# szcompressor/sz

Measured on AMD Instinct MI355X. Metric: compression GB/s (input), 512^3 float32 ABS 1e-4, higher is better.
Workload: dtype f32

## Files before the change

### sz_amd/csrc/szh_segenc.h

```cpp
#pragma once

namespace szh_se {
constexpr int NR = 4;
constexpr int INNER = 7;
constexpr int PF = 8;

struct col_t { int b0, b1, s0, s1, o0, o1, rows; };
struct seg_t {
    int bkbeg, bkend, kbeg, kend;
    int nE, E, L;
    int ka, nvec, pitch, kshift;
    int nblk, nruns;
    int lg_nvec;
};
SZH_HD int seg_pitch(int width) { int p = (width + 1) & ~1; if (((p >> 1) & 1) == 0) p += 2; return p; }
SZH_HD col_t make_col(const szh_geom3 &G, int col)
{
    col_t c;
    c.b0 = col / G.g1.num; c.b1 = col - c.b0 * G.g1.num;
    c.s0 = szh_blk_size(G.g0, c.b0); c.s1 = szh_blk_size(G.g1, c.b1); c.o0 = szh_blk_start(G.g0, c.b0); c.o1 = szh_blk_start(G.g1, c.b1);
    c.rows = c.s0 * c.s1;
    return c;
}
SZH_HD seg_t make_seg(const szh_geom3 &G, int rows, int segi, int segb, int VW)
{
    seg_t s;
    s.bkbeg = segi * segb; s.bkend = s.bkbeg + segb < G.g2.num ? s.bkbeg + segb : G.g2.num;
    s.kbeg = szh_blk_start(G.g2, s.bkbeg); s.kend = s.bkend < G.g2.num ? szh_blk_start(G.g2, s.bkend) : G.g2.count;
    s.E = G.g2.early; s.L = G.g2.late;
    int nE = G.g2.split - s.bkbeg; if (nE < 0) nE = 0; if (nE > s.bkend - s.bkbeg) nE = s.bkend - s.bkbeg;
    s.nE = nE;
    s.ka = s.kbeg / VW * VW;
    const int kb = (s.kend + VW - 1) / VW * VW;
    s.nvec = (kb - s.ka) / VW;
    s.pitch = seg_pitch(kb - s.ka); s.kshift = s.kbeg - s.ka;
    s.nblk = s.bkend - s.bkbeg; s.nruns = s.nblk * rows;
    s.lg_nvec = 0; while ((1 << s.lg_nvec) < s.nvec) ++s.lg_nvec;
    return s;
}
inline size_t seg_tile_bytes(const szh_geom3 &G, int segb, int VW)
{
    const size_t rows = (size_t)G.g0.early * G.g1.early;
    const int width = segb * G.g2.early + 2 * VW;
    return (rows * (size_t)seg_pitch(width) * 2 + 15) & ~(size_t)15;
}
inline size_t seg_pieces_per_thread(const szh_geom3 &G, int segb, int VW)
{
    const size_t rows = (size_t)G.g0.early * G.g1.early;
    const size_t nvec = ((size_t)segb * G.g2.early + 2 * VW) / VW + 1;
    size_t p2 = 1; while (p2 < nvec) p2 <<= 1;
    return (rows * p2 + 255) / 256;
}
inline size_t seg_window_words(const szh_geom3 &G, unsigned maxlen, int nrmax = NR) { return (size_t)256 * nrmax * (size_t)G.g2.early * maxlen / 32 + 8; }
}

#ifdef SZH_HIPSIM
static inline bool any_lane(bool p) { return __ballot(p ? 1 : 0) != 0ull; }
#else
__device__ __forceinline__ bool any_lane(bool p) { return __builtin_amdgcn_ballot_w64(p) != 0ull; }
#endif
__device__ __forceinline__ unsigned magic_of(unsigned d) { return d > 1u ? 0xffffffffu / d + 1u : 0u; }
__device__ __forceinline__ unsigned div_by(unsigned x, unsigned d, unsigned m) { return d > 1u ? (unsigned)(((u64)x * m) >> 32) : x; }

#define SZH_COL_HBINS 256
__global__ __launch_bounds__(256) void k_col_hist(szh_geom3 G, const uint16_t *__restrict__ codes, unsigned nbins, int rshift, int vw, unsigned *__restrict__ col_hist)
{
    SZH_DYN_SMEM(smem);
    unsigned *sh = reinterpret_cast<unsigned *>(smem);
    const unsigned R = 1u << rshift;
    for (unsigned i = threadIdx.x; i < (nbins << rshift); i += 256) sh[i] = 0;
    __syncthreads();
    const szh_se::col_t c = szh_se::make_col(G, (int)blockIdx.x);
    const int nvec = G.g2.count / vw;
    const int lane = (int)threadIdx.x & 63, wid = (int)threadIdx.x >> 6;
    const unsigned rep = threadIdx.x & (R - 1);
    const unsigned m_s1 = magic_of((unsigned)c.s1);
    for (int x = lane; x < nvec; x += 64) {
        for (int r0 = wid; r0 < c.rows; r0 += 16) {
            uint4 w[4];
#pragma unroll
            for (int q = 0; q < 4; ++q) {
                const int r = r0 + 4 * q;
                w[q] = uint4{0u, 0u, 0u, 0u};
                if (r < c.rows) {
                    const int i = (int)div_by((unsigned)r, (unsigned)c.s1, m_s1), j = r - i * c.s1;
                    const uint16_t *src = codes + (int64_t)(c.o0 + i) * G.d0 + (int64_t)(c.o1 + j) * G.d1 + x * vw;
                    if (vw == 8) w[q] = *reinterpret_cast<const uint4 *>(src);
                    else if (vw == 4) { const uint2 t = *reinterpret_cast<const uint2 *>(src); w[q].x = t.x; w[q].y = t.y; }
                    else w[q].x = src[0];
                }
            }
#pragma unroll
            for (int q = 0; q < 4; ++q) {
                if (r0 + 4 * q < c.rows) {
                    const unsigned wv[4] = {w[q].x, w[q].y, w[q].z, w[q].w};
#pragma unroll
                    for (int e = 0; e < 8; ++e) if (e < vw) { const unsigned cd = (e & 1) ? wv[e >> 1] >> 16 : wv[e >> 1] & 0xffffu; atomicAdd(&sh[(cd << rshift) + rep], 1u); }
                }
            }
        }
    }
    __syncthreads();
    for (unsigned b = threadIdx.x; b < nbins; b += 256) {
        unsigned t = 0;
        for (unsigned q = 0; q < R; ++q) t += sh[(b << rshift) + q];
        col_hist[(size_t)blockIdx.x * nbins + b] = t;
    }
}
__global__ __launch_bounds__(256) void k_hist_reduce(const unsigned *__restrict__ col_hist, unsigned nbins, int64_t ncols, unsigned *__restrict__ hist)
{
    __shared__ unsigned acc[SZH_COL_HBINS];
    for (unsigned b = threadIdx.x; b < nbins; b += 256) acc[b] = 0;
    __syncthreads();
    const unsigned tpb = 256u / nbins > 0u ? 256u / nbins : 1u;
    if (threadIdx.x < tpb * nbins) {
        const unsigned bin = threadIdx.x % nbins, lane_col = threadIdx.x / nbins;
        unsigned t = 0;
        for (int64_t col = (int64_t)blockIdx.x * tpb + lane_col; col < ncols; col += (int64_t)gridDim.x * tpb) t += col_hist[(size_t)col * nbins + bin];
        if (t) atomicAdd(&acc[bin], t);
    }
    __syncthreads();
    for (unsigned b = threadIdx.x; b < nbins; b += 256) if (acc[b]) atomicAdd(&hist[b], acc[b]);
}
__global__ __launch_bounds__(256) void k_col_bits_h(const unsigned *__restrict__ col_hist, const uint8_t *__restrict__ len, unsigned nbins, int64_t ncols, u64 *__restrict__ col_bits, u64 *__restrict__ col_zeros)
{
    __shared__ uint8_t llen[SZH_COL_HBINS];
    for (unsigned i = threadIdx.x; i < nbins; i += 256) llen[i] = len[i];
    __syncthreads();
    const int64_t e = (int64_t)blockIdx.x * 256 + threadIdx.x;
    if (e >= ncols) return;
    const unsigned *h = col_hist + (size_t)e * nbins;
    u64 bits = 0;
    for (unsigned b = 0; b < nbins; ++b) bits += (u64)h[b] * llen[b];
    col_bits[e] = bits; col_zeros[e] = h[0];
}

// ... 21 lines not shown
                    const int i = (int)div_by((unsigned)r, (unsigned)c.s1, m_s1), j = r - i * c.s1;
                    const uint16_t *src = codes + (int64_t)(c.o0 + i) * G.d0 + (int64_t)(c.o1 + j) * G.d1 + x * vw;
                    if (vw == 8) w[q] = *reinterpret_cast<const uint4 *>(src);
                    else if (vw == 4) { const uint2 t = *reinterpret_cast<const uint2 *>(src); w[q].x = t.x; w[q].y = t.y; }
                    else w[q].x = src[0];
                }
            }
#pragma unroll
            for (int q = 0; q < 4; ++q) {
                if (r0 + 4 * q < c.rows) {
                    const unsigned wv[4] = {w[q].x, w[q].y, w[q].z, w[q].w};
#pragma unroll
                    for (int e = 0; e < 8; ++e) if (e < vw) {
                        const unsigned cd = (e & 1) ? wv[e >> 1] >> 16 : wv[e >> 1] & 0xffffu;
                        bits += tab_lds ? llen[cd] : len[cd]; zeros += cd == 0u ? 1u : 0u;
                    }
                }
            }
        }
    }
    bits = wave_sum_u64(bits); const u64 z = wave_sum_u64((u64)zeros);
    if (lane == 0) { red[wid] = bits; red[4 + wid] = z; }
    __syncthreads();
    if (threadIdx.x == 0) { col_bits[blockIdx.x] = red[0] + red[1] + red[2] + red[3]; col_zeros[blockIdx.x] = red[4] + red[5] + red[6] + red[7]; }
}

__global__ __launch_bounds__(256) void k_col_bounds(const u64 *__restrict__ col_bitoff, int64_t nent, const u64 *__restrict__ total_bits, u64 bit0, unsigned *out32)
{
    const int64_t e = (int64_t)blockIdx.x * 256 + threadIdx.x;
    if (e > nent) return;
    const u64 at = bit0 + (e < nent ? col_bitoff[e] : *total_bits);
    out32[at >> 5] = 0u;
    if (e == nent) out32[(at >> 5) + 1] = 0u;
}
#define SZH_COL_SCAN_PER 8
__global__ __launch_bounds__(1024) void k_col_scan(const u64 *__restrict__ col_bits, const u64 *__restrict__ col_zeros, int nent, u64 *__restrict__ col_bitoff, u64 *__restrict__ col_zoff,
                                                   u64 *total_bits, u64 *total_zeros, u64 bit0, unsigned *out32, const u64 *__restrict__ plan = nullptr)
{
    __shared__ u64 shb[16], shz[16];
    if (plan) { if (plan[SZH_PLAN_STATUS] != 0) return; bit0 = plan[SZH_PLAN_BIT0]; }
    const int tid = (int)threadIdx.x, lane = tid & 63, wid = tid >> 6;
    const int lo = tid * SZH_COL_SCAN_PER;
    u64 vb[SZH_COL_SCAN_PER], vz[SZH_COL_SCAN_PER];
#pragma unroll
    for (int q = 0; q < SZH_COL_SCAN_PER; ++q) { const bool in = lo + q < nent; vb[q] = in ? col_bits[lo + q] : 0ull; vz[q] = in ? col_zeros[lo + q] : 0ull; }
    u64 b = 0, z = 0;
#pragma unroll
    for (int q = 0; q < SZH_COL_SCAN_PER; ++q) { b += vb[q]; z += vz[q]; }
    u64 ib = b, iz = z;
    for (int o = 1; o < 64; o <<= 1) { const u64 tb = __shfl_up(ib, o, 64), tz = __shfl_up(iz, o, 64); if (lane >= o) { ib += tb; iz += tz; } }
    if (lane == 63) { shb[wid] = ib; shz[wid] = iz; }
    __syncthreads();
    u64 baseb = 0, basez = 0, totb = 0, totz = 0;
    for (int w = 0; w < 16; ++w) { if (w < wid) { baseb += shb[w]; basez += shz[w]; } totb += shb[w]; totz += shz[w]; }
    u64 rb = baseb + ib - b, rz = basez + iz - z;
#pragma unroll
    for (int q = 0; q < SZH_COL_SCAN_PER; ++q) {
        if (lo + q < nent) { col_bitoff[lo + q] = rb; col_zoff[lo + q] = rz; out32[(bit0 + rb) >> 5] = 0u; }
        rb += vb[q]; rz += vz[q];
    }
    if (tid == 0) { *total_bits = totb; *total_zeros = totz; out32[(bit0 + totb) >> 5] = 0u; out32[((bit0 + totb) >> 5) + 1] = 0u; }
}

__global__ __launch_bounds__(1024) void k_col_zscan(const unsigned *__restrict__ col_zeros, int nent, u64 *__restrict__ col_zoff, u64 *total_zeros)
{
    __shared__ u64 shz[16];
    const int tid = (int)threadIdx.x, lane = tid & 63, wid = tid >> 6;
    const int lo = tid * SZH_COL_SCAN_PER;
    u64 vz[SZH_COL_SCAN_PER], z = 0;
#pragma unroll
    for (int q = 0; q < SZH_COL_SCAN_PER; ++q) { vz[q] = lo + q < nent ? (u64)col_zeros[lo + q] : 0ull; z += vz[q]; }
    u64 iz = z;
    for (int o = 1; o < 64; o <<= 1) { const u64 tz = __shfl_up(iz, o, 64); if (lane >= o) iz += tz; }
    if (lane == 63) shz[wid] = iz;
    __syncthreads();
    u64 basez = 0, totz = 0;
    for (int w = 0; w < 16; ++w) { if (w < wid) basez += shz[w]; totz += shz[w]; }
    u64 rz = basez + iz - z;
#pragma unroll
    for (int q = 0; q < SZH_COL_SCAN_PER; ++q) { if (lo + q < nent) col_zoff[lo + q] = rz; rz += vz[q]; }
    if (tid == 0) *total_zeros = totz;
}

template <class T, bool WIDE>
__global__ __launch_bounds__(256) void k_col_encode(szh_geom3 G, const uint16_t *__restrict__ codes, const u64 *__restrict__ table, unsigned nsym, const szh_se::seg_t *__restrict__ segs, int nseg, int vw, int nrmax,
                                                    size_t tile_bytes, unsigned win_words, const u64 *__restrict__ col_bitoff, const u64 *__restrict__ col_zoff, u64 bit0,
                                                    unsigned *out32, const T *__restrict__ data, T *__restrict__ unpred, const u64 *__restrict__ plan = nullptr)
{
    using namespace szh_se;
    if (plan) { if (plan[SZH_PLAN_STATUS] != 0) return; bit0 = plan[SZH_PLAN_BIT0]; }
    SZH_DYN_SMEM(smem);
    __shared__ u64 sh[2][4];
    __shared__ unsigned rowbase[128];
    u64 *ltab = reinterpret_cast<u64 *>(smem);
    uint16_t *tile = reinterpret_cast<uint16_t *>(smem + ((size_t)nsym + 1) * 8);
    uint16_t *nullrun = reinterpret_cast<uint16_t *>(smem + ((size_t)nsym + 1) * 8 + tile_bytes);
    unsigned *win = reinterpret_cast<unsigned *>(smem + ((size_t)nsym + 1) * 8 + tile_bytes + 16);
    const int tid = (int)threadIdx.x, lane = tid & 63, wid = tid >> 6;
    const col_t c = make_col(G, (int)blockIdx.x);
    for (unsigned i = tid; i < nsym; i += 256) ltab[i] = table[i];
    if (tid == 0) ltab[nsym] = 0;
    if (tid < 8) nullrun[tid] = (uint16_t)nsym;
    for (unsigned w = tid; w < win_words; w += 256) win[w] = 0u;
    const unsigned m_rows = magic_of((unsigned)c.rows);
    if (tid < c.rows) { const int i = tid / c.s1, j = tid - i * c.s1; rowbase[tid] = (unsigned)((int64_t)(c.o0 + i) * G.d0 + (int64_t)(c.o1 + j) * G.d1); }
    __syncthreads();
    uint4 pf[PF];
    auto fetch = [&](const seg_t &s) {
        const int lg = s.lg_nvec, mask = (1 << lg) - 1;
#pragma unroll
        for (int p = 0; p < PF; ++p) {
            const int x = p * 256 + tid, r = x >> lg, cv = x & mask;
            pf[p] = uint4{0u, 0u, 0u, 0u};
            if (r < c.rows && cv < s.nvec) {
                const uint16_t *src = codes + (size_t)rowbase[r] + (unsigned)(s.ka + cv * vw);
                if (vw == 8) pf[p] = *reinterpret_cast<const uint4 *>(src);
                else if (vw == 4) { const uint2 t = *reinterpret_cast<const uint2 *>(src); pf[p].x = t.x; pf[p].y = t.y; }
                else pf[p].x = src[0];
            }
        }
    };
    auto place = [&](const seg_t &s) {
        const int lg = s.lg_nvec, mask = (1 << lg) - 1;
        auto put_piece = [&](int r, int cv, const uint4 &w) {
            uint16_t *dst = tile + r * s.pitch + cv * vw;
            if (vw == 8) { unsigned *d = reinterpret_cast<unsigned *>(dst); d[0] = w.x; d[1] = w.y; d[2] = w.z; d[3] = w.w; }
            else if (vw == 4) { unsigned *d = reinterpret_cast<unsigned *>(dst); d[0] = w.x; d[1] = w.y; }
            else dst[0] = (uint16_t)w.x;
        };
#pragma unroll
        for (int p = 0; p < PF; ++p) { const int x = p * 256 + tid, r = x >> lg, cv = x & mask; if (r < c.rows && cv < s.nvec) put_piece(r, cv, pf[p]); }
        for (int x = PF * 256 + tid; (x >> lg) < c.rows; x += 256) {
            const int r = x >> lg, cv = x & mask;
            if (cv >= s.nvec) continue;
            const uint16_t *src = codes + (size_t)rowbase[r] + (unsigned)(s.ka + cv * vw);
            uint4 w = {0u, 0u, 0u, 0u};
            if (vw == 8) w = *reinterpret_cast<const uint4 *>(src);
            else if (vw == 4) { const uint2 t = *reinterpret_cast<const uint2 *>(src); w.x = t.x; w.y = t.y; }
            else w.x = src[0];
            put_piece(r, cv, w);
        }
    };
    seg_t s = segs[0]; s.nruns = s.nblk * c.rows;
    fetch(s);
    const u64 col_bit = bit0 + col_bitoff[blockIdx.x];
    const u64 col_word = col_bit >> 5;
    const bool col_lead = (col_bit & 31u) != 0u;
    u64 bits_done = 0, zeros_done = col_zoff[blockIdx.x];
    const int null_at = (int)(nullrun - tile);
    int par = 0;
    for (int segi = 0; segi < nseg; ++segi) {
        place(s);
        __syncthreads();
        seg_t sn = s;
        if (segi + 1 < nseg) { sn = segs[segi + 1]; sn.nruns = sn.nblk * c.rows; fetch(sn); }
        const int nrounds = (s.nruns + 256 * nrmax - 1) / (256 * nrmax);
        const int nr = (s.nruns + 256 * nrounds - 1) / (256 * nrounds);
        const int edge_k = s.nE * s.E;
        auto run_words = [&](int at, unsigned (&wv)[4]) {
            const unsigned *w = reinterpret_cast<const unsigned *>(tile + (at & ~1));
            const unsigned w0 = w[0], w1 = w[1], w2 = w[2], w3 = w[3];
            const unsigned sft = (unsigned)(at & 1) << 4;
            wv[0] = (unsigned)((((u64)w1 << 32) | w0) >> sft); wv[1] = (unsigned)((((u64)w2 << 32) | w1) >> sft);
            wv[2] = (unsigned)((((u64)w3 << 32) | w2) >> sft); wv[3] = w3 >> sft;
        };
        for (int rd = 0; rd < nrounds; ++rd, par ^= 1) {
            const int q0 = (rd * 256 + tid) * nr;
            const int bl0 = (int)div_by((unsigned)q0, (unsigned)c.rows, m_rows), row0 = q0 - bl0 * c.rows;
            unsigned sum1 = 0;
            int jn = 0;
            unsigned need7 = 0;
            if (WIDE) {
                int bl = bl0, row = row0;
                for (int j = 0; j < nr; ++j) {
                    const bool on = q0 + j < s.nruns;
                    if (!any_lane(on)) break;
                    jn = j + 1;
                    const int s2 = bl < s.nE ? s.E : s.L, koff = bl < s.nE ? bl * s.E : edge_k + (bl - s.nE) * s.L;
                    unsigned wv[4];
                    run_words(on ? row * s.pitch + s.kshift + koff : null_at, wv);
                    const bool n7 = any_lane(on && s2 == INNER);
                    if (n7) need7 |= 1u << j;
#pragma unroll
                    for (int kk = 0; kk < INNER; ++kk) {
                        unsigned cd = (kk & 1) ? wv[kk >> 1] >> 16 : wv[kk >> 1] & 0xffffu;
                        if (kk == INNER - 1) { if (!n7) continue; cd = (on && s2 == INNER) ? cd : nsym; }
                        sum1 += (unsigned)ltab[cd];
                    }
                    if (++row == c.rows) { row = 0; ++bl; }
                }
            } else {
                int bl = bl0, row = row0;
                for (int j = 0; j < nr; ++j) {
                    if (q0 + j >= s.nruns) break;
                    const int s2 = bl < s.nE ? s.E : s.L, koff = bl < s.nE ? bl * s.E : edge_k + (bl - s.nE) * s.L;
                    const uint16_t *p = tile + row * s.pitch + s.kshift + koff;
                    for (int kk = 0; kk < s2; ++kk) sum1 += (unsigned)ltab[p[kk]];
                    if (++row == c.rows) { row = 0; ++bl; }
                }
            }
            const unsigned bsum = sum1 & 0xffffu, zsum = sum1 >> 16;
            unsigned ib = bsum, iz = zsum;
            for (int o = 1; o < 64; o <<= 1) { const unsigned t = __shfl_up(ib, o, 64); if (lane >= o) ib += t; }
            if (any_lane(zsum != 0u)) for (int o = 1; o < 64; o <<= 1) { const unsigned t = __shfl_up(iz, o, 64); if (lane >= o) iz += t; }
            if (lane == 63) sh[par][wid] = (u64)ib | ((u64)iz << 32);
            __syncthreads();
            u64 base2 = 0, tot2 = 0;
#pragma unroll
            for (int w = 0; w < 4; ++w) { const u64 t = sh[par][w]; if (w < wid) base2 += t; tot2 += t; }
            const unsigned tot = (unsigned)tot2, ex = (unsigned)base2 + ib - bsum;
            const u64 gbit = col_bit + bits_done;
            const unsigned lead = (unsigned)(gbit & 31u);
            const unsigned nwords = (lead + tot + 31u) >> 5;
            {
                const unsigned bitpos = lead + ex;
                unsigned wpos = bitpos >> 5, nb = bitpos & 31u;
                u64 acc = 0;
                auto put = [&](unsigned le, unsigned cw) {
                    acc = (acc << (le & 63u)) | cw;
                    nb += le & 0xffffu;
                    if (nb >= 32u) { atomicOr(&win[wpos], (unsigned)(acc >> (nb - 32u))); ++wpos; nb -= 32u; }
                };
                if (WIDE) {
                    int bl = bl0, row = row0;
                    if (any_lane(bsum != 0u))
                    for (int j = 0; j < jn; ++j) {
                        const bool on = q0 + j < s.nruns;
                        const int s2 = bl < s.nE ? s.E : s.L, koff = bl < s.nE ? bl * s.E : edge_k + (bl - s.nE) * s.L;
                        unsigned wv[4];
                        run_words(on ? row * s.pitch + s.kshift + koff : null_at, wv);
                        const bool n7 = (need7 >> j) & 1u;
#pragma unroll
                        for (int kk = 0; kk < INNER; ++kk) {
                            unsigned cd = (kk & 1) ? wv[kk >> 1] >> 16 : wv[kk >> 1] & 0xffffu;
                            if (kk == INNER - 1) { if (!n7) continue; cd = (on && s2 == INNER) ? cd : nsym; }
                            const u64 en = ltab[cd];
                            put((unsigned)en, (unsigned)(en >> 32));
                        }
                        if (++row == c.rows) { row = 0; ++bl; }
                    }
                } else if (bsum) {
                    int bl = bl0, row = row0;
                    for (int j = 0; j < nr; ++j) {
                        if (q0 + j >= s.nruns) break;
                        const int s2 = bl < s.nE ? s.E : s.L, koff = bl < s.nE ? bl * s.E : edge_k + (bl - s.nE) * s.L;
                        const uint16_t *p = tile + row * s.pitch + s.kshift + koff;
                        for (int kk = 0; kk < s2; ++kk) { const u64 en = ltab[p[kk]]; put((unsigned)en, (unsigned)(en >> 32)); }
                        if (++row == c.rows) { row = 0; ++bl; }
                    }
                }
                if (bsum && nb) atomicOr(&win[wpos], (unsigned)(acc << (32u - nb)));
            }
            if (zsum) {
                u64 zat = zeros_done + (unsigned)(base2 >> 32) + iz - zsum;
                int bl = bl0, row = row0;
                for (int j = 0; j < nr; ++j) {
                    if (q0 + j >= s.nruns) break;
                    const int s2 = bl < s.nE ? s.E : s.L, koff = bl < s.nE ? bl * s.E : edge_k + (bl - s.nE) * s.L;
                    const uint16_t *p = tile + row * s.pitch + s.kshift + koff;
                    const T *drow = data + (size_t)rowbase[row] + (unsigned)(s.kbeg + koff);
                    for (int kk = 0; kk < s2; ++kk) if (p[kk] == 0) unpred[zat++] = drow[kk];
                    if (++row == c.rows) { row = 0; ++bl; }
                }
            }
            const bool last_round = rd + 1 == nrounds && segi + 1 == nseg;
            if (tot) {
                __syncthreads();
                const bool partial = ((lead + tot) & 31u) != 0u;
                const unsigned nout = (partial && !last_round) ? nwords - 1 : nwords;
                const u64 w0 = gbit >> 5;
                unsigned keep = 0u;
                if (tid == 0 && partial && !last_round) { keep = win[nwords - 1]; if (nwords > 1) win[nwords - 1] = 0u; }
                for (unsigned w = tid; w < nout; w += 256) {
                    const unsigned x = __builtin_bswap32(win[w]);
                    win[w] = w == 0 ? keep : 0u;
                    const bool shared = (col_lead && w0 + w == col_word) || (w == nwords - 1 && last_round && partial);
                    if (shared) { if (x) atomicOr(&out32[w0 + w], x); }
                    else out32[w0 + w] = x;
                }
                bits_done += tot;
            } else if (rd + 1 == nrounds && segi + 1 < nseg) __syncthreads();
            zeros_done += tot2 >> 32;
        }
        s = sn;
    }
}

__global__ __launch_bounds__(256) void k_col_zeros(szh_geom3 G, const uint16_t *__restrict__ blk, unsigned *__restrict__ col_zeros)
{
    __shared__ unsigned red[4];
    const szh_se::col_t c = szh_se::make_col(G, (int)blockIdx.x);
    const int64_t base = szh_code_base01(G, c.b0, c.b1), len = (int64_t)c.rows * G.g2.count;
    const int head = (int)(base & 7);
    const int64_t ngroups = (head + len + 7) / 8;
    unsigned z = 0;
    for (int64_t g = threadIdx.x; g < ngroups; g += 256) {
        const uint4 w = *reinterpret_cast<const uint4 *>(blk + (base - head) + g * 8);
        const unsigned wv[4] = {w.x, w.y, w.z, w.w};
#pragma unroll
        for (int e = 0; e < 8; ++e) {
            const int64_t at = g * 8 + e - head;
            const unsigned cd = (e & 1) ? wv[e >> 1] >> 16 : wv[e >> 1] & 0xffffu;
            z += (at >= 0 && at < len && cd == 0u) ? 1u : 0u;
        }
    }
    z = wave_sum_u32(z);
    if ((threadIdx.x & 63) == 0) red[threadIdx.x >> 6] = z;
    __syncthreads();
    if (threadIdx.x == 0) col_zeros[blockIdx.x] = red[0] + red[1] + red[2] + red[3];
}
template <class T>
__global__ __launch_bounds__(256) void k_col_unpack(szh_geom3 G, const uint16_t *__restrict__ blk, uint16_t *__restrict__ nat, const szh_se::seg_t *__restrict__ segs, int nseg, int vw,
                                                    const u64 *__restrict__ col_zoff, const T *__restrict__ unpred, u64 ucap, T *__restrict__ out)
{
    using namespace szh_se;
    SZH_DYN_SMEM(smem);
    __shared__ u64 sh[8];
    __shared__ unsigned rowbase[128];
    uint16_t *L = reinterpret_cast<uint16_t *>(smem);
    const int tid = (int)threadIdx.x;
    const col_t c = make_col(G, (int)blockIdx.x);
    if (tid < c.rows) { const int i = tid / c.s1, j = tid - i * c.s1; rowbase[tid] = (unsigned)((int64_t)(c.o0 + i) * G.d0 + (int64_t)(c.o1 + j) * G.d1); }
    const int64_t col_base = szh_code_base01(G, c.b0, c.b1);
    u64 zeros_done = col_zoff[blockIdx.x];
    for (int segi = 0; segi < nseg; ++segi) {
        const seg_t s = segs[segi];
        const int klen = s.kend - s.kbeg, total = c.rows * klen;
        const int64_t start = col_base + (int64_t)c.rows * s.kbeg;
        const int head = (int)(start & 7), ngroups = (head + total + 7) / 8;
        __syncthreads();
        for (int g = tid; g < ngroups; g += 256) *reinterpret_cast<uint4 *>(L + g * 8) = *reinterpret_cast<const uint4 *>(blk + (start - head) + (int64_t)g * 8);
        __syncthreads();
        const uint16_t *B = L + head;
        const int esz = c.rows * s.E, lsz = c.rows * s.L, eregion = s.nE * esz;
// ... 63 lines not shown
```

### sz_amd/csrc/szhip_sz21.inc

```
static bool book_declines(unsigned rec_status, unsigned long long plan_status, int test_switch) { return rec_status != 0 || plan_status != 0 || test_switch != 0; }

static int hist_rshift(unsigned intervals, size_t cap_bins) { int r = 0; while (r < 6 && ((size_t)intervals << (r + 1)) <= cap_bins) ++r; return r; }

struct sz21_plan {
    bool use_beam = false;
    bool segenc = false;
    bool seghist = false;
    bool dev_book = false;
    bool sliced = false;
    int slices_req = 1;
    int se_vw = 1, se_segb = 0, se_nseg = 0, se_nrmax = szh_se::NR; size_t se_tile = 0;
    int sh_rshift = 0;
    bool revise(unsigned enc_maxlen) { if (!segenc || enc_maxlen <= 32) return false; segenc = false; seghist = false; return true; }
};
template <class T>
sz21_plan sz21_make_plan(const szhip_ctx *ctx, const szh_geom3 &G, unsigned intervals, size_t reg_count, bool beam_ok, bool overlap, bool feed, size_t meta_len)
{
    sz21_plan P;
    const int64_t n = G.n;
    P.use_beam = !overlap && beam_ok;
    const int segenc_sw = tune_int("SZ_HIP_SEGENC", 1);
    P.segenc = G.ndim == 3 && segenc_sw != 0 && (!feed || segenc_sw == 2);
    P.se_vw = (G.g2.count % 8) == 0 ? 8 : ((G.g2.count % 4) == 0 ? 4 : 1);
    if (P.segenc) {
        bool ok = intervals < 65536 && (double)n < 4.0e9;
        if ((int64_t)G.g0.late * G.g1.late * G.g2.late < 32) ok = false;
        const size_t fixed = ((size_t)intervals + 1) * 8 + 16 + szh_se::seg_window_words(G, 32) * 4 + 64;
        const size_t lds_cap = (size_t)63 * 1024, want = (size_t)std::max(4, tune_int("SZ_HIP_SEG_TILE_KB", 14)) * 1024;
        if (ok && fixed + szh_se::seg_tile_bytes(G, 1, P.se_vw) > lds_cap) ok = false;
        if (ok) {
            const size_t budget = std::min(lds_cap - fixed, std::max(want, szh_se::seg_tile_bytes(G, 1, P.se_vw)));
            int sb = 1;
            while (sb < G.g2.num && szh_se::seg_tile_bytes(G, sb + 1, P.se_vw) <= budget && szh_se::seg_pieces_per_thread(G, sb + 1, P.se_vw) <= (size_t)szh_se::PF) ++sb;
            sb = (G.g2.num + (G.g2.num + sb - 1) / sb - 1) / ((G.g2.num + sb - 1) / sb);
            if (const int f = tune_int("SZ_HIP_SEG_SEGB", 0)) sb = std::max(1, std::min(f, sb));
            P.se_segb = sb;
            P.se_nseg = (G.g2.num + sb - 1) / sb;
            P.se_tile = szh_se::seg_tile_bytes(G, sb, P.se_vw);
            const int rows_typ = (2 * G.g0.split > G.g0.num ? G.g0.early : G.g0.late) * (2 * G.g1.split > G.g1.num ? G.g1.early : G.g1.late);
            const int runs_typ = std::max(1, sb * rows_typ), rounds_typ = (runs_typ + 256 * szh_se::NR - 1) / (256 * szh_se::NR);
            P.se_nrmax = std::max(1, std::min(szh_se::NR, (runs_typ + 256 * rounds_typ - 1) / (256 * rounds_typ)));
            if ((double)G.g0.num * G.g1.num >= 2.0e9) ok = false;
        }
        P.segenc = ok;
    }
    P.seghist = P.segenc && intervals <= SZH_COL_HBINS && tune_int("SZ_HIP_SEGHIST", 1) != 0;
    if (P.seghist) P.sh_rshift = hist_rshift(intervals, 4096);
    P.dev_book = P.segenc && reg_count == 0 && !ctx->no_dev_book && tune_int("SZ_HIP_DEV_BOOK", 0) != 0 && G.g0.num * G.g1.num <= 1024 * SZH_COL_SCAN_PER &&
                 tune_int("SZ_HIP_SEG_SCAN1", 1) != 0 && meta_len + 8 + 4 + sizeof(T) + 1 + sizeof(T) <= 3072;
    P.slices_req = tune_int("SZ_HIP_SLICES", ctx->gate ? tune_int("SZ_HIP_SLICES_POOL", 2) : 4);
    P.sliced = P.use_beam && P.slices_req > 1 && !P.seghist;
    return P;
}

template <class T>
struct sz21_call {
    static constexpr int is_double = sizeof(T) == 8;
    static constexpr int64_t LINE = 128 / (int64_t)sizeof(T);
    szhip_ctx *const ctx; const szhip_params *const prm; const unsigned char *meta; const size_t meta_len; const int out_on_device; unsigned char **const out; size_t *const out_size;
    const double eb_in; const T eb; const hipStream_t st;
    const bool two_d;
    const szh_geom3 G; const int ncoef, ncols; const int64_t n, nb;
    const double t_begin = now_ms(); double host_ms = 0;
    const int tp_on = tune_int("SZ_HIP_TIMING", 0); double tp_t[32]; const char *tp_n[32]; int tp_k = 0;
    szhip_stats S;
    const T *d_in = nullptr; u64 *sm = nullptr; T *d_coef = nullptr; uint8_t *d_lor = nullptr; uint16_t *d_nat = nullptr, *d_blk = nullptr; unsigned *d_hist = nullptr, *h_hist = nullptr;
    T noise = 0; bool fit_tile = false; int ft_nseg = 0;
    size_t ind_bytes = 0; unsigned char *ind_bits = nullptr; u64 *nreg_h = nullptr, *minmax_h = nullptr;
    unsigned intervals = 0; int use_mean = 0; T mean = 0; size_t reg_count = 0;
    std::vector<unsigned char> meta_own;
    sz21_plan P;
    unsigned *tile_done = nullptr; size_t beam_words = 0;
    int perm_segb = 1, perm_nseg = 1; size_t perm_lds = 0;
    std::vector<szh_se::seg_t> se_segs; std::vector<u64> tab_code; std::vector<uint8_t> tab_len;
    unsigned enc_maxlen = 0; bool enc32 = false; size_t lds_e32 = 0;
    unsigned char *hdr = nullptr; size_t pre_len = 0, sections_total = 0, hdr_len = 0, unpred_bytes = 0, total_len = 0; u64 total_bits = 0, total_unpred = 0;
    u64 h_small[SM_COUNT];
    bool synced = false;
    szhost_coeffs cf;
    size_t sec_len[4] = {0, 0, 0, 0};
    std::vector<std::thread> section_threads;
    std::atomic<int> section_failed{0};
    std::vector<unsigned char> all_reg_keep;
    std::vector<uint32_t> blk_of_rank;
    size_t chain_done[4] = {0, 0, 0, 0};
    size_t chain_avail = 0;
    double chain_t0[4] = {0, 0, 0, 0}, chain_t1[4] = {0, 0, 0, 0};
    bool overlap = false, feed = false, two_pieces = false;
    fed_call_guard fed_guard;
    T *hcoef = nullptr;
    bool pool_busy = false;
    bool cf_own = false;
    sz21_call(szhip_ctx *c, size_t r0, size_t r1, size_t r2, double eb_, const szhip_params *p, const unsigned char *m, size_t ml, int ood, unsigned char **o, size_t *os)
        : ctx(c), prm(p), meta(m), meta_len(ml), out_on_device(ood), out(o), out_size(os), eb_in(eb_), eb((T)eb_), st(c->stream), two_d(r0 == 0),
          G(r0 == 0 ? szh_make_geom2((int)r1, (int)r2) : szh_make_geom3((int)r0, (int)r1, (int)r2)), ncoef(r0 == 0 ? 3 : 4), ncols(G.g0.num * G.g1.num), n(G.n), nb(G.nblocks)
    {
        memset(&S, 0, sizeof(S)); memset(&cf, 0, sizeof(cf));
        S.n_elements = (uint64_t)n; S.n_blocks = (uint64_t)nb;
    }
    ~sz21_call() {
        join_sections();
        if (ctx->chain_pool) ctx->chain_pool->disarm();
        if (cf_own) for (int e = 0; e < 4; ++e) { cf.codes[e] = nullptr; cf.unpred[e] = nullptr; }
        szhost_coeffs_free(&cf);
    }
    void join_sections() {
        for (auto &x : section_threads) if (x.joinable()) x.join();
        if (pool_busy && ctx->chain_pool) { ctx->chain_pool->wait_all(); pool_busy = false; }
    }
    void TP(const char *nm) { if (tp_on && tp_k < 32) { tp_t[tp_k] = now_ms() - t_begin; tp_n[tp_k++] = nm; } }
    void print_trace() const { if (tp_on) { for (int i = 0; i < tp_k; ++i) fprintf(stderr, "%s %.2f | ", tp_n[i], tp_t[i]); fprintf(stderr, "\n"); } }
    bool is_lorenzo(int64_t bb) const { return (ind_bits[bb >> 3] >> (7 - (bb & 7))) & 1; }
    size_t count_lorenzo(int64_t bb, int64_t b_end) const {
        size_t ones = 0;
        for (; bb < b_end && (bb & 7); ++bb) ones += is_lorenzo(bb);
        for (; bb + 64 <= b_end; bb += 64) { uint64_t w8; memcpy(&w8, ind_bits + (bb >> 3), 8); ones += (size_t)__builtin_popcountll(w8); }
        for (; bb < b_end; ++bb) ones += is_lorenzo(bb);
        return ones;
    }
    size_t chains_done() const {
        size_t p = reg_count;
        for (int e = 0; e < ncoef; ++e) { const size_t d = __atomic_load_n(&chain_done[e], __ATOMIC_ACQUIRE); if (d < p) p = d; }
        return p;
    }
    int launch_fit(hipStream_t s_, int um, T mn) {
// ... 439 lines not shown
                if ((++spins & 127u) == 0) {
                    const hipError_t q = hipEventQuery(ctx->ev[3]);
                    if (q == hipSuccess) { sweep_over = true; break; }
                    if (q != hipErrorNotReady) HIPCHK(q);
                }
            }
            if (b0_hi > b0_done) {
                const int64_t h_lo = hist_first, h_hi = b0_hi >= G.g0.num ? (int64_t)n : ((int64_t)rows_need * G.d0) / 8 * 8;
                hist_first = h_hi;
                const int grid = (int)std::min<int64_t>(((h_hi - h_lo) / 8 + 255) / 256 + 1, 2048);
                if (h_hi > h_lo) hipLaunchKernelGGL(k_hist_u16, dim3(grid), dim3(256), hist_lds, ctx->stream2, (const uint16_t *)d_nat, h_hi, intervals, rshift, use_lds, d_hist, h_lo);
                if (!P.segenc) launch_permute(ctx->stream3, b0_done * G.g1.num, (b0_hi - b0_done) * G.g1.num);
                HIPCHK(hipGetLastError());
                b0_done = b0_hi;
            }
        }
        HIPCHK(hipMemcpyAsync(h_hist, d_hist, (size_t)intervals * 4, hipMemcpyDeviceToHost, ctx->stream2));
        HIPCHK(hipEventRecord(ctx->ev_fit, ctx->stream2));
        if (!P.segenc) TRY(scan_col_zeros(ctx->stream3));
        HIPCHK(hipEventRecord(ctx->ev_perm, ctx->stream3));
        return SZHIP_OK;
    }
    int hist_and_order() {
        TRY(ensure(ctx, ctx->hist, (size_t)(65536 + 8192) * 4 + 64));
        d_hist = (unsigned *)ctx->hist.p;
        TRY(ensure_pinned(ctx, (size_t)intervals * 4 + 64));
        h_hist = (unsigned *)ctx->pinned;
        if (P.seghist) {
            TRY(ensure(ctx, ctx->seg_hist, (size_t)ncols * intervals * 4));
            HIPCHK(hipMemsetAsync(d_hist, 0, (size_t)intervals * 4, st));
            hipLaunchKernelGGL(k_col_hist, dim3((unsigned)ncols), dim3(256), ((size_t)intervals * 4) << P.sh_rshift, st, G, (const uint16_t *)d_nat, intervals, P.sh_rshift, P.se_vw, (unsigned *)ctx->seg_hist.p);
            hipLaunchKernelGGL(k_hist_reduce, dim3((unsigned)std::min<int64_t>(64, ncols)), dim3(256), 0, st, (const unsigned *)ctx->seg_hist.p, intervals, (int64_t)ncols, d_hist);
            HIPCHK(hipGetLastError());
            if (!P.dev_book) {
                HIPCHK(hipMemcpyAsync(h_hist, d_hist, (size_t)intervals * 4, hipMemcpyDeviceToHost, st));
                HIPCHK(hipEventRecord(ctx->ev_fit, st));
            }
        } else if (!P.sliced) TRY(launch_hist());
        TRY(ensure(ctx, ctx->col_zeros, (size_t)ncols * 4));
        TRY(ensure(ctx, ctx->col_zeros64, (size_t)ncols * 8));
        TRY(ensure(ctx, ctx->col_off, (size_t)ncols * 8));
        if (P.sliced) TRY(hist_and_order_sliced());
        else if (!P.segenc) TRY(permute_all());
        return SZHIP_OK;
    }
    unsigned char *put_front(unsigned char *q) const {
        memcpy(q, meta, meta_len); q += meta_len;
        szhost_put_u64be(q, (uint64_t)n); q += 8;
        szhost_put_u32be(q, (uint32_t)G.block_size); q += 4;
        if (is_double) szhost_put_f64be(q, (double)eb); else szhost_put_f32be(q, (float)eb);
        return q + sizeof(T);
    }
    int upload_segments() {
        se_segs.resize((size_t)P.se_nseg);
        for (int q = 0; q < P.se_nseg; ++q) se_segs[(size_t)q] = szh_se::make_seg(G, 1, q, P.se_segb, P.se_vw);
        TRY(ensure(ctx, ctx->seg_tab, se_segs.size() * sizeof(szh_se::seg_t)));
        HIPCHK(hipMemcpyAsync(ctx->seg_tab.p, se_segs.data(), se_segs.size() * sizeof(szh_se::seg_t), hipMemcpyHostToDevice, st));
        return SZHIP_OK;
    }
    template <class F>
    int pack_columns(unsigned char *d_stream, u64 base_bits, const u64 *d_plan, unsigned maxlen, F &&between) {
        const int64_t nent = (int64_t)ncols;
        TRY(ensure(ctx, ctx->seg_bits, (size_t)nent * 8)); TRY(ensure(ctx, ctx->seg_zeros, (size_t)nent * 8));
        TRY(ensure(ctx, ctx->seg_bitoff, (size_t)nent * 8)); TRY(ensure(ctx, ctx->seg_zoff, (size_t)nent * 8));
        u64 *const bits = (u64 *)ctx->seg_bits.p, *const zeros = (u64 *)ctx->seg_zeros.p, *const bitoff = (u64 *)ctx->seg_bitoff.p, *const zoff = (u64 *)ctx->seg_zoff.p;
        const size_t lb = intervals <= 16384 ? (size_t)intervals : 16;
        if (P.seghist) hipLaunchKernelGGL(k_col_bits_h, dim3((unsigned)((nent + 255) / 256)), dim3(256), 0, st, (const unsigned *)ctx->seg_hist.p, (const uint8_t *)ctx->len_tab.p, intervals, nent, bits, zeros);
        else hipLaunchKernelGGL(k_col_bits, dim3((unsigned)nent), dim3(256), lb, st, G, (const uint16_t *)d_nat, (const uint8_t *)ctx->len_tab.p, intervals, P.se_vw, bits, zeros);
        if (nent <= 1024 * SZH_COL_SCAN_PER && tune_int("SZ_HIP_SEG_SCAN1", 1))
            hipLaunchKernelGGL(k_col_scan, dim3(1), dim3(1024), 0, st, (const u64 *)bits, (const u64 *)zeros, (int)nent, bitoff, zoff, sm + SM_TOTAL_BITS, sm + SM_TOTAL_UNPRED, base_bits, (unsigned *)d_stream, d_plan);
        else {
            TRY(scan_u64(ctx, (const u64 *)bits, nent, bitoff, sm + SM_TOTAL_BITS));
            TRY(scan_u64(ctx, (const u64 *)zeros, nent, zoff, sm + SM_TOTAL_UNPRED));
            hipLaunchKernelGGL(k_col_bounds, dim3((unsigned)((nent + 1 + 255) / 256)), dim3(256), 0, st, (const u64 *)bitoff, nent, (const u64 *)(sm + SM_TOTAL_BITS), base_bits, (unsigned *)d_stream);
        }
        HIPCHK(hipGetLastError());
        TRY(between());
        const unsigned win = (unsigned)szh_se::seg_window_words(G, std::max(1u, maxlen), P.se_nrmax);
        const size_t lds = ((size_t)intervals + 1) * 8 + P.se_tile + 16 + (size_t)win * 4;
        auto encode = [&](auto kernel) {
            hipLaunchKernelGGL(kernel, dim3((unsigned)nent), dim3(256), lds, st, G, (const uint16_t *)d_nat, (const u64 *)ctx->code_tab.p, intervals, (const szh_se::seg_t *)ctx->seg_tab.p, P.se_nseg, P.se_vw,
                               P.se_nrmax, P.se_tile, win, (const u64 *)bitoff, (const u64 *)zoff, base_bits, (unsigned *)d_stream, d_in, (T *)ctx->unpred.p, d_plan);
        };
        if (G.g2.num >= 2 && G.g2.early <= szh_se::INNER && G.g2.late >= szh_se::INNER - 1) encode(k_col_encode<T, true>);
        else encode(k_col_encode<T, false>);
        HIPCHK(hipGetLastError());
        return SZHIP_OK;
    }
    int enqueue_readback() {
        HIPCHK(hipEventRecord(ctx->ev[4], st));
        TP("encode launched");
        HIPCHK(hipMemcpyAsync(h_small, sm, SM_COUNT * 8, hipMemcpyDeviceToHost, st));
        return SZHIP_OK;
    }
    int deliver(unsigned char *d_stream, size_t len, bool in_place) {
        if (out_on_device == 2) {
            if (!*out || *out_size < len) FAIL(SZHIP_ERR_ARG, "caller's device buffer too small (%zu < %zu)", *out_size, len);
            if (!in_place) { HIPCHK(hipMemcpyAsync(*out, d_stream, len, hipMemcpyDeviceToDevice, st)); synced = false; }
            if (!synced) HIPCHK(hipStreamSynchronize(st));
        } else if (out_on_device) {
            if (!synced) HIPCHK(hipStreamSynchronize(st));
            *out = d_stream;
        } else {
            unsigned char *h = (unsigned char *)malloc(len ? len : 1);
            if (!h) FAIL(SZHIP_ERR_INTERNAL, "out of host memory");
            const int rc_copy = staged_copy(ctx, h, d_stream, len, false);
            if (rc_copy != SZHIP_OK) { free(h); return rc_copy; }
            *out = h;
        }
        *out_size = len;
        synced = true;
        return SZHIP_OK;
    }
    int check_final(bool declined, unsigned book_status, u64 bits, u64 unpred) {
        if ((unsigned)h_small[SM_ERR] == 2) { ctx->coef_late = true; FAIL(SZHIP_ERR_INTERNAL, "wavefront kernel: the regression coefficients did not arrive"); }
        if ((unsigned)h_small[SM_ERR] != 0) { ctx->wave_timeout = true; FAIL(SZHIP_ERR_INTERNAL, "wavefront kernel: halo wait timed out"); }
        if (declined) {
            ctx->book_declined = true;
            snprintf(ctx->err, sizeof(ctx->err), "device code book declined (status %u)", book_status);
            return SZHIP_ERR_INTERNAL;
        }
        if ((bits > 0 && h_small[SM_TOTAL_BITS] != bits) || h_small[SM_TOTAL_UNPRED] != unpred)
            FAIL(SZHIP_ERR_INTERNAL, "entropy stage mismatch (bits %llu vs %llu, unpredictable %llu vs %llu)", (unsigned long long)h_small[SM_TOTAL_BITS],
                 (unsigned long long)bits, (unsigned long long)h_small[SM_TOTAL_UNPRED], (unsigned long long)unpred);
        return SZHIP_OK;
    }
    void finish_stats(size_t len, u64 unpred, int packing, int book_on_device) {
        float ms = 0;
        hipEventElapsedTime(&ms, ctx->ev[0], ctx->ev[1]); S.ms_prequant = ms;
        hipEventElapsedTime(&ms, ctx->ev[2], ctx->ev[3]); S.ms_quant = ms;
        hipEventElapsedTime(&ms, ctx->ev[3], ctx->ev[4]); S.ms_entropy = ms;
        S.n_unpred = unpred; S.ms_host = host_ms; S.ms_total = now_ms() - t_begin; S.out_bytes = len; S.packing = packing; S.book_on_device = book_on_device;
    }
    int encode_with_device_book() {
        const size_t bk_front = meta_len + 8 + 4 + sizeof(T), bk_mid = 1 + sizeof(T);
        if (!P.seghist) HIPCHK(hipStreamWaitEvent(st, ctx->ev_fit, 0));
        if (!ctx->book_pin) HIPCHK(hipHostMalloc((void **)&ctx->book_pin, 4096, hipHostMallocDefault));
        unsigned char *const blob = (unsigned char *)ctx->book_pin + 256;
        unsigned char *const mid = put_front(blob);
        mid[0] = (unsigned char)use_mean; memcpy(mid + 1, &mean, sizeof(T));
        const size_t plan_fixed = bk_front + 12 + bk_mid + ind_bytes + 8;
        const size_t tree_cap = 1 + (size_t)9 * (2 * SZH_BOOK_CAP - 1);
        const size_t unpred_cap = std::min((size_t)n * sizeof(T), (size_t)n * sizeof(T) / 4 + 65536);
        const bool in_place = out_on_device == 2 && *out && *out_size >= plan_fixed + tree_cap + 64 && ((uintptr_t)*out & 15) == 0 && tune_int("SZ_HIP_OUT_IN_PLACE", 1);
        const size_t stream_cap = in_place ? *out_size : plan_fixed + tree_cap + (size_t)n * sizeof(T) + 65536;
        if (!in_place) TRY(ensure(ctx, ctx->stream_buf, stream_cap));
        unsigned char *d_stream = in_place ? (unsigned char *)*out : (unsigned char *)ctx->stream_buf.p;
        TRY(ensure(ctx, ctx->book_stage, bk_front + bk_mid)); TRY(ensure(ctx, ctx->book_tree, tree_cap)); TRY(ensure(ctx, ctx->book_rec, 32 + SZH_PLAN_COUNT * 8));
        TRY(ensure(ctx, ctx->code_tab, (size_t)intervals * 8)); TRY(ensure(ctx, ctx->len_tab, (size_t)intervals));
        TRY(ensure(ctx, ctx->unpred, unpred_cap + 64));
        szh_book_rec *const d_rec = (szh_book_rec *)ctx->book_rec.p;
        u64 *const d_plan = (u64 *)((char *)ctx->book_rec.p + 32);
        HIPCHK(hipMemcpyAsync(ctx->book_stage.p, blob, bk_front + bk_mid, hipMemcpyHostToDevice, st));
        hipLaunchKernelGGL(k_huff_book, dim3(1), dim3(256), 0, st, (const unsigned *)d_hist, intervals, SZH_BOOK_TAB_SEG, (unsigned char *)ctx->book_tree.p, (unsigned)tree_cap,
                           (u64 *)ctx->code_tab.p, (uint8_t *)ctx->len_tab.p, d_rec, d_plan, (u64)plan_fixed, (unsigned)sizeof(T), (u64)stream_cap, (u64)unpred_cap);
        HIPCHK(hipGetLastError());
        TRY(upload_segments());
        TRY(pack_columns(d_stream, 0, (const u64 *)d_plan, 32u, [&]() -> int {
            hipLaunchKernelGGL(k_book_tail, dim3((unsigned)std::min<size_t>(64, (plan_fixed + tree_cap + 255) / 256)), dim3(256), 0, st, d_stream, (const unsigned char *)ctx->book_stage.p, (unsigned)bk_front,
                               (unsigned)bk_mid, intervals, (const unsigned char *)ctx->lor_bits.p, ind_bytes, (const unsigned char *)ctx->book_tree.p, (const szh_book_rec *)d_rec, (const u64 *)d_plan);
            return SZHIP_OK;
        }));
        hipLaunchKernelGGL((k_book_unpred<T>), dim3((unsigned)std::min<size_t>(256, (unpred_cap / sizeof(T) + 255) / 256)), dim3(256), 0, st, d_stream, (const T *)ctx->unpred.p, (const szh_book_rec *)d_rec, (const u64 *)d_plan);
        HIPCHK(hipGetLastError());
        TRY(enqueue_readback());
        HIPCHK(hipMemcpyAsync(ctx->book_pin, ctx->book_rec.p, 32 + SZH_PLAN_COUNT * 8, hipMemcpyDeviceToHost, st));
        HIPCHK(hipStreamSynchronize(st));
        synced = true;
// ... 589 lines not shown
```

Baseline: 375.7.

## Pack each run's Huffman codes into a 64-bit word and deposit with few atomics

In the wide segment encoder, each run's up to seven Huffman codes are concatenated into a 64-bit accumulator during the sizing pass and kept in registers. The emit pass then deposits each run with at most three atomicOr operations into the LDS window instead of re-reading the tile and emitting code by code. Runs longer than 64 bits fall back to the original per-code path. This adds register pressure (NR u64 plus sums) and a divergent overflow path. It is enabled by default through a tuning flag.

Result: no change. 375.2 (-0.1%).

```diff
diff --git a/sz_amd/csrc/szh_segenc.h b/sz_amd/csrc/szh_segenc.h
--- a/sz_amd/csrc/szh_segenc.h
+++ b/sz_amd/csrc/szh_segenc.h
@@ -52,6 +52,11 @@
     return (rows * p2 + 255) / 256;
 }
 inline size_t seg_window_words(const szh_geom3 &G, unsigned maxlen, int nrmax = NR) { return (size_t)256 * nrmax * (size_t)G.g2.early * maxlen / 32 + 8; }
+SZH_HD void run_deposit(u64 acc, unsigned len, unsigned sh, unsigned &a0, unsigned &a1, unsigned &a2)
+{
+    const u64 v = len ? acc << (64u - len) : 0ull;
+    a0 = (unsigned)(v >> 32) >> sh; a1 = (unsigned)(v >> sh); a2 = (unsigned)((v << 32) >> sh);
+}
 }
 
 #ifdef SZH_HIPSIM
@@ -239,7 +244,7 @@
     if (tid == 0) *total_zeros = totz;
 }
 
-template <class T, bool WIDE>
+template <class T, bool WIDE, bool RUNW = false>
 __global__ __launch_bounds__(256) void k_col_encode(szh_geom3 G, const uint16_t *__restrict__ codes, const u64 *__restrict__ table, unsigned nsym, const szh_se::seg_t *__restrict__ segs, int nseg, int vw, int nrmax,
                                                     size_t tile_bytes, unsigned win_words, const u64 *__restrict__ col_bitoff, const u64 *__restrict__ col_zoff, u64 bit0,
                                                     unsigned *out32, const T *__restrict__ data, T *__restrict__ unpred, const u64 *__restrict__ plan = nullptr)
@@ -327,7 +332,35 @@
             unsigned sum1 = 0;
             int jn = 0;
             unsigned need7 = 0;
-            if (WIDE) {
+            u64 racc[NR]; unsigned rsum[NR];
+            if (WIDE && RUNW) {
+                static_assert(!RUNW || WIDE, "run words: only where a run is read as four words");
+                int bl = bl0, row = row0;
+#pragma unroll
+                for (int j = 0; j < NR; ++j) { racc[j] = 0ull; rsum[j] = 0u; }
+#pragma unroll
+                for (int j = 0; j < NR; ++j) {
+                    if (j >= nr) break;
+                    const bool on = q0 + j < s.nruns;
+                    if (!any_lane(on)) break;
+                    jn = j + 1;
+                    const int s2 = bl < s.nE ? s.E : s.L, koff = bl < s.nE ? bl * s.E : edge_k + (bl - s.nE) * s.L;
+                    unsigned wv[4];
+                    run_words(on ? row * s.pitch + s.kshift + koff : null_at, wv);
+                    const bool n7 = any_lane(on && s2 == INNER);
+                    u64 a = 0ull; unsigned rs = 0u;
+#pragma unroll
+                    for (int kk = 0; kk < INNER; ++kk) {
+                        unsigned cd = (kk & 1) ? wv[kk >> 1] >> 16 : wv[kk >> 1] & 0xffffu;
+                        if (kk == INNER - 1) { if (!n7) continue; cd = (on && s2 == INNER) ? cd : nsym; }
+                        const u64 en = ltab[cd];
+                        a = (a << ((unsigned)en & 63u)) | (en >> 32);
+                        rs += (unsigned)en;
+                    }
+                    racc[j] = a; rsum[j] = rs; sum1 += rs;
+                    if (++row == c.rows) { row = 0; ++bl; }
+                }
+            } else if (WIDE) {
                 int bl = bl0, row = row0;
                 for (int j = 0; j < nr; ++j) {
                     const bool on = q0 + j < s.nruns;
@@ -378,7 +411,42 @@
                     nb += le & 0xffffu;
                     if (nb >= 32u) { atomicOr(&win[wpos], (unsigned)(acc >> (nb - 32u))); ++wpos; nb -= 32u; }
                 };
-                if (WIDE) {
+                if (WIDE && RUNW) {
+                    if (any_lane(bsum != 0u)) {
+                        unsigned bp = bitpos, ovf = 0u;
+#pragma unroll
+                        for (int j = 0; j < NR; ++j) {
+                            if (j >= jn) break;
+                            const unsigned len = rsum[j] & 0xffffu;
+                            if (len <= 64u) {
+                                unsigned a0, a1, a2;
+                                run_deposit(racc[j], len, bp & 31u, a0, a1, a2);
+                                unsigned *w = win + (bp >> 5);
+                                if (a0) atomicOr(w, a0);
+                                if (a1) atomicOr(w + 1, a1);
+                                if (a2) atomicOr(w + 2, a2);
+                            } else ovf |= 1u << j;
+                            bp += len;
+                        }
+                        if (any_lane(ovf != 0u)) {
+                            unsigned at = bitpos;
+#pragma unroll 1
+                            for (int j = 0; j < jn; ++j) {
+                                const unsigned rs = j == 0 ? rsum[0] : j == 1 ? rsum[1] : j == 2 ? rsum[2] : rsum[NR - 1];
+                                static_assert(NR == 4, "the selection above");
+                                if ((ovf >> j) & 1u) {
+                                    const int q = q0 + j, bl = (int)div_by((unsigned)q, (unsigned)c.rows, m_rows), row = q - bl * c.rows;
+                                    const int s2 = bl < s.nE ? s.E : s.L, koff = bl < s.nE ? bl * s.E : edge_k + (bl - s.nE) * s.L;
+                                    const uint16_t *p = tile + row * s.pitch + s.kshift + koff;
+                                    wpos = at >> 5; nb = at & 31u; acc = 0;
+                                    for (int kk = 0; kk < s2; ++kk) { const u64 en = ltab[p[kk]]; put((unsigned)en, (unsigned)(en >> 32)); }
+                                    if (nb) atomicOr(&win[wpos], (unsigned)(acc << (32u - nb)));
+                                }
+                                at += rs & 0xffffu;
+                            }
+                        }
+                    }
+                } else if (WIDE) {
                     int bl = bl0, row = row0;
                     if (any_lane(bsum != 0u))
                     for (int j = 0; j < jn; ++j) {
@@ -406,7 +474,7 @@
                         if (++row == c.rows) { row = 0; ++bl; }
                     }
                 }
-                if (bsum && nb) atomicOr(&win[wpos], (unsigned)(acc << (32u - nb)));
+                if (!(WIDE && RUNW) && bsum && nb) atomicOr(&win[wpos], (unsigned)(acc << (32u - nb)));
             }
             if (zsum) {
                 u64 zat = zeros_done + (unsigned)(base2 >> 32) + iz - zsum;
diff --git a/sz_amd/csrc/szhip_sz21.inc b/sz_amd/csrc/szhip_sz21.inc
--- a/sz_amd/csrc/szhip_sz21.inc
+++ b/sz_amd/csrc/szhip_sz21.inc
@@ -11,6 +11,7 @@
     int slices_req = 1;
     int se_vw = 1, se_segb = 0, se_nseg = 0, se_nrmax = szh_se::NR; size_t se_tile = 0;
     int sh_rshift = 0;
+    bool se_runwords = true;
     bool revise(unsigned enc_maxlen) { if (!segenc || enc_maxlen <= 32) return false; segenc = false; seghist = false; return true; }
 };
 template <class T>
@@ -41,6 +42,7 @@
             const int runs_typ = std::max(1, sb * rows_typ), rounds_typ = (runs_typ + 256 * szh_se::NR - 1) / (256 * szh_se::NR);
             P.se_nrmax = std::max(1, std::min(szh_se::NR, (runs_typ + 256 * rounds_typ - 1) / (256 * rounds_typ)));
             if ((double)G.g0.num * G.g1.num >= 2.0e9) ok = false;
+            P.se_runwords = tune_int("SZ_HIP_SEG_RUNWORDS", 1) != 0;
         }
         P.segenc = ok;
     }
@@ -646,8 +648,10 @@
             hipLaunchKernelGGL(kernel, dim3((unsigned)nent), dim3(256), lds, st, G, (const uint16_t *)d_nat, (const u64 *)ctx->code_tab.p, intervals, (const szh_se::seg_t *)ctx->seg_tab.p, P.se_nseg, P.se_vw,
                                P.se_nrmax, P.se_tile, win, (const u64 *)bitoff, (const u64 *)zoff, base_bits, (unsigned *)d_stream, d_in, (T *)ctx->unpred.p, d_plan);
         };
-        if (G.g2.num >= 2 && G.g2.early <= szh_se::INNER && G.g2.late >= szh_se::INNER - 1) encode(k_col_encode<T, true>);
-        else encode(k_col_encode<T, false>);
+        const bool wide = G.g2.num >= 2 && G.g2.early <= szh_se::INNER && G.g2.late >= szh_se::INNER - 1;
+        if (wide && P.se_runwords) encode(k_col_encode<T, true, true>);
+        else if (wide) encode(k_col_encode<T, true, false>);
+        else encode(k_col_encode<T, false, false>);
         HIPCHK(hipGetLastError());
         return SZHIP_OK;
     }
```
